# falcon-computing/bwa-flow

Measured on AMD Instinct MI355X. Metric: million reads/sec (2×150 bp PE) end-to-end align; SW-extend GCUPS at 1/2/4/8 MI355X, higher is better.
Workload: dtype int32

## Files before the change

bwa-flow_amd/csrc/capi.hip:

```cpp
#include <hip/hip_runtime.h>
#include <string.h>

#include <algorithm>
#include <chrono>
#include <cstdio>
#include <mutex>
#include <new>
#include <string>
#include <thread>
#include <vector>

#include "batch_host.h"
#include "ctx.h"
#include "engine.h"
#include "regpost.h"

using namespace bwagpu;

namespace {


__global__ void side_probe_spin(uint64_t ticks) {
  const uint64_t t0 = __builtin_amdgcn_s_memrealtime();
  while (__builtin_amdgcn_s_memrealtime() - t0 < ticks) __builtin_amdgcn_s_sleep(8);
// ... 118 lines not shown
  std::string why;
  if (!make_opt(opt, &ctx->opt, &why)) {
    delete ctx;
    return BWAGPU_E_INVAL;
  }
  ctx->device = device;
  ctx->opt_b = opt->b;
  ctx->ext_form = set_ext_form(-1);
  ctx->ext_short = ext_short_default();
  ctx->ext_short_fill = ext_short_fill_default();
  ctx->light_pack = light_pack_default();
  ctx->ungapped = ungapped_default();
  ctx->ungapped_right = ungapped_right_default();
  ctx->emu_finish = emu_finish_default();
  ctx->fused_launches = fused_launches_default();
  *made = ctx;
  HIPC(hipSetDevice(device), "hipSetDevice");
  HIPC(hipMalloc(&ctx->d_ann_off, sizeof(int64_t) * bns->n_seqs), "hipMalloc(ann_offset)");
  HIPC(hipMalloc(&ctx->d_ann_len, sizeof(int32_t) * bns->n_seqs), "hipMalloc(ann_len)");
  HIPC(hipMemcpy(ctx->d_ann_off, bns->ann_offset, sizeof(int64_t) * bns->n_seqs, hipMemcpyHostToDevice),
       "upload ann_offset");
  HIPC(hipMemcpy(ctx->d_ann_len, bns->ann_len, sizeof(int32_t) * bns->n_seqs, hipMemcpyHostToDevice),
       "upload ann_len");
  for (auto& s : ctx->slot) {
    HIPC(hipEventCreate(&s.ev0), "hipEventCreate");
    HIPC(hipEventCreate(&s.ev1), "hipEventCreate");
    HIPC(hipEventCreate(&s.ev2), "hipEventCreate");
    HIPC(hipEventCreate(&s.ev3), "hipEventCreate");
  }
  ctx->ref.l_pac = bns->l_pac;
// ... 174 lines not shown
  }();
  a.emu_strict = emu_strict;
  a.light_pack = ctx->light_pack;
  a.emu_finish = ctx->emu_finish;
  a.out = d_out;
  a.out_n = d_n;
  a.stats = d_stats;
  SpecStreams ss;
  HIPC(choose_side(ctx, s, st, &ss), "side stream");
  a.lq_bound = lq_max;
  const int tb = tb_bytes_for(ctx->opt, std::max(lq_max, 1));
  ss.form = ctx->ext_form;
  ss.short_q = ctx->ext_short;
  ss.short_fill = ctx->ext_short_fill;
  ss.fused = ctx->fused_launches;
  ss.pool = ctx->prof_ev.empty() ? nullptr : ctx->prof_ev.data();
  ss.pool_n = (int)ctx->prof_ev.size();
  ss.pool_used = &ctx->prof_used;
  HIPC(launch_spec_clear(a, db.n_reads, db.n_seeds, st), "spec clear");
  HIPC(launch_spec_chain2aln(ctx->opt, ctx->ref, db, a, tb, lq_max, st, ss), "spec chain2aln launch");
  return BWAGPU_OK;
}

}

int bwagpu::enqueue_chain2aln(bwagpu_ctx_t* ctx, Slot& s, const DevBatch& db, int lq_max, bwagpu_alnreg_t* d_out,
                              int32_t* d_n, int64_t* d_stats, hipStream_t st) {
  if (!use_read_kernels()) return enqueue_spec(ctx, s, db, lq_max, d_out, d_n, d_stats, st);
  ChainWin* win = nullptr;
  bwagpu_seed_t* prog = nullptr;
// ... 534 lines not shown

int bwagpu_ctx_emu_finish(bwagpu_ctx_t* ctx, int on) {
  if (!ctx) return BWAGPU_E_INVAL;
  const int prev = ctx->emu_finish;
  if (on >= 0) ctx->emu_finish = on ? 1 : 0;
  return prev;
}

int bwagpu_ctx_fused_launches(bwagpu_ctx_t* ctx, int mask) {
  if (!ctx) return BWAGPU_E_INVAL;
  const int prev = ctx->fused_launches;
  if (mask >= 0) ctx->fused_launches = mask & 7;
  return prev;
}

int bwagpu_debug_spec_finish(bwagpu_ctx_t* ctx, void* stream, int64_t* out) {
  if (!ctx || !out) return BWAGPU_E_INVAL;
  int32_t c[SPC_WORDS];
  if (int rc = spec_ctr_words(ctx, stream, c)) return rc;
  out[0] = c[SPC_FIN_NAR];
  out[1] = c[SPC_FIN_WIDE];
  out[2] = c[SPC_LIST_N];
  out[3] = c[SPC_LIGHT_N];
  return BWAGPU_OK;
}

int bwagpu_ctx_row_bound(bwagpu_ctx_t* ctx, int on) {
  if (!ctx) return BWAGPU_E_INVAL;
  const int prev = ctx->opt.row_bound;
  if (on >= 0) ctx->opt.row_bound = on ? 1 : 0;
  return prev;
}

int bwagpu_debug_ext_kernel(bwagpu_ctx_t* ctx, int32_t lq_max) {
  if (!ctx || lq_max < 1 || lq_max > BWAGPU_MAX_READ_LEN) return BWAGPU_E_INVAL;
  return ext_kernel_for(ctx->opt, ctx->ext_form, tb_bytes_for(ctx->opt, lq_max));
}

// ... 54 lines not shown
```

bwa-flow_amd/csrc/ctx.h:

```cpp
#pragma once
#include <hip/hip_runtime.h>
#include <stdint.h>

#include <algorithm>
#include <atomic>
#include <chrono>
#include <mutex>
#include <string>
#include <type_traits>
#include <vector>

#include "bwagpu.h"
#include "chain.h"
#include "engine.h"
#include "rescue.h"
#include "seed.h"
#include "stage_host.h"
#include "task_host.h"

namespace bwagpu {

inline std::atomic<int64_t> g_live_bufs{0}, g_live_bytes{0};

template <bool kPinned>
// ... 100 lines not shown
  bwagpu::DevOpt opt{};
  bwagpu::DevRef ref{};
  bool own_pac = false;
  void* d_pac = nullptr;
  int64_t* d_ann_off = nullptr;
  int32_t* d_ann_len = nullptr;
  int watchdog_ms = 10000;
  int ext_form = 0;
  int ext_short = 0;
  int light_pack = 0;
  int ext_short_fill = 0;
  int ungapped = 1;
  int ungapped_right = 1;
  int emu_finish = 1;
  int fused_launches = 5;
  Slot slot[BWAGPU_NUM_SLOTS];
  hipStream_t dev_stream[BWAGPU_NUM_SLOTS] = {};
  Slot dev_scratch[BWAGPU_NUM_SLOTS];
  DevBuf ex_tasks, ex_list, ex_q, ex_t, ex_res, ex_stats;
  DevBuf a2_tasks, a2_q, a2_t, a2_out, a2_scratch, a2_lists, a2_counts, a2_boff;
  DevBuf r2_tasks, r2_q, r2_out, r2_cig, r2_md, r2_lists, r2_z, r2_stats;
  DevBuf r2d_keys, r2d_lists, r2d_tab, r2d_z, r2d_sums;
  HostBuf r2d_htab;
  hipEvent_t r2d_done = nullptr, r2d_ev[2] = {};
  bool r2d_pending = false, r2d_timing = false, r2d_timed = false;
  double r2d_wait_ms = 0, r2d_call_ms = 0;
  int32_t r2d_jobs = 0;
  static constexpr int kA2Streams = 4;
  hipStream_t a2_st[kA2Streams] = {};
  hipEvent_t a2_fork = nullptr, a2_join[kA2Streams] = {};
// ... 198 lines not shown
```

bwa-flow_amd/csrc/engine.h:

```cpp
#pragma once
#include <hip/hip_runtime.h>
#include <stdint.h>

#include "bwagpu.h"
#include "bwagpu_debug.h"
#include "pure.h"
#include "spec_plan.h"
#include "ungapped.h"

namespace bwagpu {

struct ReadDesc {
  int64_t qoff;
  int32_t rd;
  int32_t lq;
  int32_t c0;
  int32_t nch;
  int32_t s0;
  int32_t ns;
};

struct ChainWin {
  int64_t lo, hi;
};
// ... 163 lines not shown
  int ext_prefetch;
  bwagpu_alnreg_t* out;
  int32_t* out_n;
  int64_t* stats;
};
struct SpecStreams {
  hipStream_t side = nullptr;
  hipEvent_t fork = nullptr, join = nullptr;
  hipEvent_t* pool = nullptr;
  int pool_n = 0;
  int* pool_used = nullptr;
  int form = 0;
  int short_q = 0;
  int short_fill = 0;
  int fused = 0;
};
enum {
  kFuseSort = 1,
  kFuseSettle = 2,
  kFuseHeavy = 4,
};
int fused_launches_default();
int ungapped_default();
int ungapped_right_default();
int emu_finish_default();
int set_ext_form(int form);
int ext_short_default();
int ext_short_fill_default();
int light_pack_default();
int ext_kernel_for(const DevOpt& o, int form, int tb_bytes);
hipError_t launch_spec_clear(const SpecArgs& a, int n_reads, int n_seeds, hipStream_t st);
hipError_t launch_spec_chain2aln(const DevOpt& o, const DevRef& ref, const DevBatch& b, const SpecArgs& a,
                                 int tb_bytes, int lq_max, hipStream_t st, const SpecStreams& ss);
size_t spec_select_lds(int tb_bytes);
int spec_redo_cap(int tb_bytes);

struct StreamTask {
// ... 27 lines not shown
```

bwa-flow_amd/csrc/spec.hip:

```cpp
#include "spec_dev.h"

namespace bwagpu {

__device__ uint32_t* g_trace = nullptr;
hipError_t set_trace_spec(void* p) { return hipMemcpyToSymbol(HIP_SYMBOL(g_trace), &p, sizeof(p)); }


__global__ void __launch_bounds__(256) spec_chain_kernel(DevOpt o, DevRef ref, DevBatch b, SpecArgs a) {
  sel_prio();
  const int c = blockIdx.x * blockDim.x + threadIdx.x;
  bool task = false, longc = false;
  int bin = 0, s0 = 0;
  if (c < b.n_chains) {
    const int rd = a.chain_read[c];
    s0 = b.chain_seed_off[c];
    const int ns = b.chain_seed_off[c + 1] - s0;
    const int lq = (int)(b.seq_off[rd + 1] - b.seq_off[rd]);
    if (ns <= 0) {
      a.win[c] = ChainWin{0, 0};
    } else {
      int64_t wlo = ref.l_pac << 1, whi = 0;
      longc = ns > kOrderLane;
      if (!longc) {
        uint64_t key[kOrderLane];
#pragma unroll
        for (int t = 0; t < kOrderLane; ++t) {
          key[t] = ~0ull;
          if (t < ns) {
            const bwagpu_seed_t v = b.seeds[s0 + t];
// ... 21 lines not shown
      } else {
        if (!longc) a.win[c] = ChainWin{wlo, whi};
        task = lq <= a.lq_bound;
        bin = spec_bin(lq);
      }
    }
  }
#pragma unroll
  for (int k = 0; k < kSpecBins; ++k) {
    const int p = wave_append(&a.ctr[SPC_CNT + k], task && bin == k);
    if (p >= 0) a.tasks[(size_t)k * b.n_chains + p] = make_int2(s0, c);
  }
  const int p = wave_append(&a.ctr[SPC_LONG_N], longc);
  if (p >= 0) a.longc[p] = c;
}

__global__ void __launch_bounds__(256) spec_reads_kernel(DevBatch b, SpecArgs a) {
  sel_prio();
  const int rd = blockIdx.x * blockDim.x + threadIdx.x;
  bool heavy = false;
  int ns = 0;
  if (rd < b.n_reads) {
    const int lq = (int)(b.seq_off[rd + 1] - b.seq_off[rd]);
    if (lq > a.lq_bound) atomicOr((unsigned long long*)&a.stats[ST_ERR], (unsigned long long)ERR_LEN);
    ReadDesc d;
    d.qoff = b.seq_off[rd];
    d.rd = rd;
    d.lq = lq;
    d.c0 = b.read_chain_off[rd];
    d.nch = b.read_chain_off[rd + 1] - d.c0;
    d.s0 = b.chain_seed_off[d.c0];
    d.ns = b.chain_seed_off[d.c0 + d.nch] - d.s0;
    a.rdesc[rd] = d;
    for (int c = d.c0; c < d.c0 + d.nch; ++c) a.chain_read[c] = rd;
    heavy = d.ns > kSelLight || d.nch > kSelLight;
    ns = d.ns;
  }
  const int p = wave_append(&a.ctr[SPC_HEAVY_N], heavy);
  if (p >= 0) {
    a.heavy[p] = rd;
    const long long words = 2 * tri_off(ns);
    int woff = -1, col = 0;
    if (ns <= kSelMatMaxSeeds) {
      const long long o = (long long)atomicAdd(reinterpret_cast<unsigned long long*>(&a.ctr[SPC_MATW64]),
                                               (unsigned long long)words);
      if (o + words <= a.mat_words) {
        woff = (int)o;
        col = atomicAdd(&a.ctr[SPC_HCOLS], ns);
        for (int i = 0; i < ns; ++i) a.colent[col + i] = p;
      }
    }
    a.hinfo[p] = make_int4(rd, woff, col, ns);
  }
}

constexpr int kOrderBlocks = 1024;
constexpr int kOrderLds = 4096;
__device__ __forceinline__ uint64_t order_key(const bwagpu_seed_t* sd, int i) {
  return (uint64_t)(uint32_t)sd[i].score << 32 | (uint32_t)i;
}
__global__ void __launch_bounds__(256) spec_order_kernel(DevOpt o, DevRef ref, DevBatch b, SpecArgs a) {
  sel_prio();
  __shared__ uint64_t keys[kOrderLds];
  __shared__ int64_t wred[2][4];
  const int tid = (int)threadIdx.x;
  const int n_long = __hip_atomic_load(&a.ctr[SPC_LONG_N], __ATOMIC_RELAXED, __HIP_MEMORY_SCOPE_AGENT);
  for (int gi = (int)blockIdx.x; gi < n_long; gi += (int)gridDim.x) {
// ... 2006 lines not shown
}
int emu_finish_default() {
  static const int on = [] {
    const char* e = getenv("BWAGPU_EMU_FINISH");
    return !(e && e[0] == '0');
  }();
  return on;
}
int fused_launches_default() {
  static const int m = [] {
    const char* e = getenv("BWAGPU_FUSED_LAUNCHES");
    return (e && e[0] ? atoi(e) : 5) & 7;
  }();
  return m;
}
int ext_short_fill_default() {
  static const int f = [] {
    const char* e = getenv("BWAGPU_EXT_SHORT_FILL");
    return std::min(std::max(e && e[0] ? atoi(e) : BWAGPU_EXT_SHORT_FILL_DEFAULT, 0), 100000);
  }();
  return f;
}


static void launch_sort(const ExtBin& k, const ExtRound& r, int bin0, int nbins, int short_q, int short_fill) {
  if (k.phased) launch_side_sort(r, bin0, nbins, short_q, short_fill);
  else launch_task_sort(r, bin0, nbins);
}
static void launch_ext_bin(const ExtBin& k, const ExtRound& r, int list, const ExtPlan& p, int short_fill) {
  if (k.family == SIDE4) launch_side_bin(k, r, list, p, short_fill);
// ... 15 lines not shown
  const bool prof = ss.pool && *ss.pool_used + 2 <= ss.pool_n;
  if (prof) (void)hipEventRecord(ss.pool[*ss.pool_used], st);
  launch_ext_bin(plan.bin[0], r, l + 0, plan, ss.short_fill);
  if (prof) {
    (void)hipEventRecord(ss.pool[*ss.pool_used + 1], st);
    *ss.pool_used += 2;
  }
  if (!bin1) return;
  launch_ext_bin(plan.bin[1], r, l + 1, plan, ss.short_fill);
  if (bin2) launch_task_long(r, l + 2);
}

hipError_t launch_spec_chain2aln(const DevOpt& o, const DevRef& ref, const DevBatch& b, const SpecArgs& a,
                                 int tb_bytes, int lq_max, hipStream_t st, const SpecStreams& ss) {
  if (b.n_reads == 0) return hipSuccess;
  hipLaunchKernelGGL(spec_reads_kernel, dim3((b.n_reads + 255) / 256), dim3(256), 0, st, b, a);
  if (b.n_chains) {
    hipLaunchKernelGGL(spec_chain_kernel, dim3((b.n_chains + 255) / 256), dim3(256), 0, st, o, ref, b, a);
    hipLaunchKernelGGL(spec_order_kernel, dim3(kOrderBlocks), dim3(256), 0, st, o, ref, b, a);
  }
  if (b.n_chains) {
    launch_ext_round(o, ref, b, a, 0, tb_bytes, lq_max, st, ss);
    launch_select<SEL_EMULATE>(o, ref, b, a, tb_bytes, st, ss);
    launch_ext_round(o, ref, b, a, 1, tb_bytes, lq_max, st, ss);
  }
  SpecArgs af = a;
  if (!b.n_chains) af.emu_finish = 0;
  launch_select<SEL_FINAL>(o, ref, b, af, tb_bytes, st, ss);
  if (b.n_chains && lq_max > kSpecBinLen[0] && !a.emu_strict) launch_ext_round(o, ref, b, a, 2, tb_bytes, lq_max, st, ss);
  if (b.n_chains) launch_select<SEL_REDO>(o, ref, b, a, tb_bytes, st, ss);
  return hipGetLastError();
}

__global__ void __launch_bounds__(256) spec_clear_kernel(SpecArgs a, int nr, int ns) {
  const int t0 = (int)(blockIdx.x * 256 + threadIdx.x), nt = (int)(gridDim.x * 256);
// ... 32 lines not shown
```

bwa-flow_amd/csrc/spec_side.hip:

```cpp
#include "side_sort.h"
#include "spec_dev.h"

namespace bwagpu {


struct UngSide {
  const uint8_t* rd;
  int64_t x0;
  int p0, d, qlen, lq;
};
__device__ __forceinline__ UngSeg ung_pass(const UngSide& s, const DevRef& ref, int base, const int8_t* mat,
                                           const int8_t* mat8, int max_mat) {
  const int last = min(base + 15, s.qlen - 1), cnt = last - base + 1;
  const int64_t two1 = (ref.l_pac << 1) - 1, pac_bytes = (ref.l_pac >> 2) + 1;
  const int64_t xa = s.x0 + (int64_t)s.d * base, xb = s.x0 + (int64_t)s.d * last;
  const bool rev = xa >= ref.l_pac;
  const int64_t fa = rev ? two1 - xa : xa, fb = rev ? two1 - xb : xb;
  UngSeg g;
  if (s.lq >= 16 && pac_bytes >= 8 && (xb >= ref.l_pac) == rev) {
    const int qa = s.p0 + s.d * base;
    const int ws = min(max(min(qa, qa + 15 * s.d), 0), s.lq - 16);
    const int64_t b0 = min(min(fa, fb) >> 2, pac_bytes - 8);
    uint64_t q[2], tw;
    __builtin_memcpy(q, s.rd + ws, 16);
// ... 380 lines not shown
    }
    __syncthreads();
#pragma unroll
    for (int m = 0; m < kPer; ++m) {
      if (kl[m] >= 0) foL[cnt[0][kl[m]] + rl[m]] = ft[m];
      if (kr[m] >= 0) foR[cnt[1][kr[m]] + rr[m]] = ft[m];
    }
    __syncthreads();
    for (int k = threadIdx.x; k < 2 * 256; k += 256) cnt[k >> 8][k & 255] = 0;
    __syncthreads();
  }
  if (threadIdx.x < 2 && ung[threadIdx.x])
    atomicAdd(&a.ctr[(threadIdx.x ? SPC_UNG_Q : SPC_UNG_N) + round], ung[threadIdx.x]);
}

__global__ void __launch_bounds__(256) spec_settle_right_kernel(DevOpt o, DevBatch b, SpecArgs a, int round, int bin0) {
  sel_prio();
  __shared__ int tot[2];
  __shared__ unsigned long long cel;
  if (threadIdx.x < 2) tot[threadIdx.x] = 0;
  if (threadIdx.x == 0) cel = 0;
  __syncthreads();
  const int list = round * kSpecBins + bin0 + (int)blockIdx.y;
  const int n = __hip_atomic_load(&a.ctr[SPC_CNT + list], __ATOMIC_RELAXED, __HIP_MEMORY_SCOPE_AGENT);
  const size_t off = spec_list_off(list, b.n_chains, b.n_seeds);
  int sides = 0, bases = 0;
  unsigned long long cells = 0;
  for (int i = (int)(blockIdx.x * 256 + threadIdx.x); i < n; i += (int)gridDim.x * 256) {
    const UngTask t = a.ungt[off + i];
    const int qb = (int)(t.qls & 1023u), ln = (int)((t.qls >> 10) & 1023u), lq = (int)(t.qls >> 20);
    if (!side_lists(a, off + i, qb, lq - qb - ln).late) continue;
    SeedExt e = a.ext[t.pos];
    settle_right(o, e, t.rbeg, qb, ln, lq, a.ung[off + i].side[1].s);
    e.w = max(e.w, o.w);
    e.calls += 2;
    a.ext[t.pos] = e;
    ++sides;
    bases += lq - qb - ln;
    cells += (unsigned long long)e.cells;
  }
  if (sides) {
    atomicAdd(&tot[0], sides);
    atomicAdd(&tot[1], bases);
    atomicAdd(&cel, cells);
  }
  __syncthreads();
  if (threadIdx.x < 2 && tot[threadIdx.x])
    atomicAdd(&a.ctr[(threadIdx.x ? SPC_UNGR_Q : SPC_UNGR_N) + round], tot[threadIdx.x]);
  if (threadIdx.x == 0 && cel) atomicAdd(reinterpret_cast<unsigned long long*>(a.ctr + SPC_SPEC64), cel);
}

struct SideTask {
  int64_t rbeg, qoff, rb;
  int32_t pos, dlo, dhi, qbeg, len, lq;
  int32_t tt, score, h0, truesc, qb, aw0, cells, rows, calls, pad_;
};
static_assert(sizeof(SideTask) <= 96, "SideTask layout");
typedef __attribute__((address_space(3))) SideTask LdsS;
#define SIDE_FIELDS(X) X(rbeg) X(qoff) X(rb) X(pos) X(dlo) X(dhi) X(qbeg) X(len) X(lq) X(tt) X(score) X(h0) \
  X(truesc) X(qb) X(aw0) X(cells) X(rows) X(calls)
__device__ __forceinline__ void spark(LdsS* p, const SideTask& t) {
#define X(f) p->f = t.f;
  SIDE_FIELDS(X)
#undef X
// ... 253 lines not shown
    if (hb) {
      SideTask t = sload(sb);
      if (side_advance<G, RIGHT>(t, o, a, xb, tlb, spec_cells)) hb = false;
      else spark(sb, t);
    }
#ifdef BWAGPU_OCC_DIAG
    tw[3] += __builtin_amdgcn_s_memtime() - c3;
#endif
  }
  return started;
}

template <int G, int PMAX, bool K8, bool RIGHT>
__global__ void __launch_bounds__(kBlock) spec_side4_kernel(DevOpt o, DevRef ref, DevBatch b, SpecArgs a, int list,
                                                            int tb_bytes, int wave_lds, int short_q, int tb_short,
                                                            int short_fill) {
  extern __shared__ __attribute__((aligned(16))) uint8_t lds[];
  uint8_t* const wlds = lds + (size_t)(threadIdx.x >> 6) * (size_t)wave_lds;
  const int n = uni(__hip_atomic_load(&a.ctr[(RIGHT ? SPC_RCNT : SPC_LCNT) + list], __ATOMIC_RELAXED,
                                      __HIP_MEMORY_SCOPE_AGENT));
  const FatTask* fl = (RIGHT ? a.ftaskR : a.ftask) + spec_list_off(list, b.n_chains, b.n_seeds);
  constexpr bool kShort = G == 16 && K8;
  int n_long = n;
  if constexpr (kShort) {
    if (short_q > 0) {
      n_long = min(n, uni(__hip_atomic_load(&a.ctr[(RIGHT ? SPC_RLONG : SPC_LLONG) + list], __ATOMIC_RELAXED,
                                            __HIP_MEMORY_SCOPE_AGENT)));
      const long long slots = (long long)gridDim.x * (kBlock / 64) * (128 / kShortG);
      if ((long long)(n - n_long) * 100 < slots * short_fill) n_long = n;
    }
  }
// ... 19 lines not shown
#endif
      if ((threadIdx.x & (kShortG - 1)) == 0 && ns) {
        atomicAdd(&a.ctr[SPC_SHORT_N], ns);
        atomicAdd(reinterpret_cast<unsigned long long*>(a.ctr + SPC_SPEC64), (unsigned long long)cells_s);
      }
    }
  }
#ifdef BWAGPU_OCC_DIAG
  if ((threadIdx.x & 63) == 0) {
    for (int k = 0; k < 8; ++k) atomicAdd(reinterpret_cast<unsigned long long*>(a.ctr + 32) + k, occ[k]);
    for (int k = 0; k < 4; ++k) atomicAdd(reinterpret_cast<unsigned long long*>(a.ctr + 48) + k, tw[k]);
  }
#endif
  if ((threadIdx.x & (G - 1)) == 0 && spec_cells)
    atomicAdd(reinterpret_cast<unsigned long long*>(a.ctr + SPC_SPEC64), (unsigned long long)spec_cells);
}


void launch_side_sort(const ExtRound& r, int bin0, int nbins, int short_q, int short_fill) {
  const int fuse = (r.ss.fused & kFuseSort) ? 1 : 0;
  if (r.a.ung)
    hipLaunchKernelGGL(spec_ungapped_kernel, dim3(512, nbins), dim3(256), 0, r.st, r.o, r.ref, r.b, r.a, r.round, bin0,
                       short_fill == 0 ? short_q : 0, fuse);
  if (!(fuse && r.a.ung)) hipLaunchKernelGGL(spec_sort2_count, dim3(256, nbins), dim3(256), 0, r.st, r.b, r.a, r.round, bin0);
  if (!fuse)
    hipLaunchKernelGGL(spec_sort2_scan, dim3(2 * nbins), dim3(256), 0, r.st, r.a, r.round, bin0, nbins, short_q);
  hipLaunchKernelGGL(spec_sort2_scatter, dim3(256, nbins), dim3(256), 0, r.st, r.o, r.b, r.a, r.round, bin0, short_q,
                     fuse);
}

template <int G, int PMAX, bool K8>
static void launch_side_pair(const ExtRound& r, int list, const ExtPlan& p, int short_fill) {
  const size_t lds = (size_t)(kBlock / 64) * p.wave_lds;
  const int nb = resident_blocks(spec_side4_kernel<G, PMAX, K8, false>, lds);
  const int gr = r.round == 2 ? std::min(nb, 64) : std::min(nb, ext2_grid(1 << 30, true));
  if (!(G == 16 && K8)) short_fill = 0;
  hipLaunchKernelGGL((spec_side4_kernel<G, PMAX, K8, false>), dim3(gr), dim3(kBlock), lds, r.st, r.o, r.ref, r.b, r.a,
                     list, r.tb_bytes, (int)p.wave_lds, p.short_q, p.tb_short, short_fill);
  const bool beside = r.a.ungt && r.ss.side && (r.ss.fused & kFuseSettle);
  if (beside) {
    (void)hipEventRecord(r.ss.fork, r.st);
    (void)hipStreamWaitEvent(r.ss.side, r.ss.fork, 0);
    hipLaunchKernelGGL(spec_settle_right_kernel, dim3(256, 1), dim3(256), 0, r.ss.side, r.o, r.b, r.a, r.round,
                       list % kSpecBins);
    (void)hipEventRecord(r.ss.join, r.ss.side);
  } else if (r.a.ungt) {
    hipLaunchKernelGGL(spec_settle_right_kernel, dim3(256, 1), dim3(256), 0, r.st, r.o, r.b, r.a, r.round,
                       list % kSpecBins);
  }
  hipLaunchKernelGGL((spec_side4_kernel<G, PMAX, K8, true>), dim3(gr), dim3(kBlock), lds, r.st, r.o, r.ref, r.b, r.a,
                     list, r.tb_bytes, (int)p.wave_lds, p.short_q, p.tb_short, short_fill);
  if (beside) (void)hipStreamWaitEvent(r.st, r.ss.join, 0);
}

void launch_side_bin(const ExtBin& k, const ExtRound& r, int list, const ExtPlan& p, int short_fill) {
  switch (ext_key(k.family, k.G, k.PMAX, k.K8)) {
    case ext_key(SIDE4, 16, 10, true): return launch_side_pair<16, 10, true>(r, list, p, short_fill);
    case ext_key(SIDE4, 32, 5, true): return launch_side_pair<32, 5, true>(r, list, p, short_fill);
    case ext_key(SIDE4, 32, 8, false): return launch_side_pair<32, 8, false>(r, list, p, short_fill);
    default: abort();
  }
}

}
```

bwa-flow_amd/python/bwagpu/abi.py:

```python
from __future__ import annotations

import ctypes as C
import os

import numpy as np

HERE = os.path.dirname(os.path.abspath(__file__))
PKG_ROOT = os.path.normpath(os.path.join(HERE, "..", ".."))
REPO_ROOT = os.path.normpath(os.path.join(PKG_ROOT, ".."))
LIB_DIR = os.path.join(PKG_ROOT, "lib")

ABI_VERSION = 1
OK, E_INVAL, E_NOMEM, E_DEVICE, E_HANG, E_RESULTS, E_UNSUPPORTED, E_NODEVICE = range(8)
ERR_NAMES = {
    OK: "OK", E_INVAL: "E_INVAL", E_NOMEM: "E_NOMEM", E_DEVICE: "E_DEVICE", E_HANG: "E_HANG",
    E_RESULTS: "E_RESULTS", E_UNSUPPORTED: "E_UNSUPPORTED", E_NODEVICE: "E_NODEVICE",
}
MAX_READ_LEN = 1023
NUM_SLOTS = 4

SEED_DTYPE = np.dtype([("rbeg", "<i8"), ("qbeg", "<i4"), ("len", "<i4"), ("score", "<i4"),
                       ("pad", "<i4")])
ALNREG_DTYPE = np.dtype([
    ("rb", "<i8"), ("re", "<i8"), ("qb", "<i4"), ("qe", "<i4"), ("rid", "<i4"), ("score", "<i4"),
# ... 178 lines not shown
    "bwagpu_set_device_read_len": (C.c_int, [_VP, C.c_int32]),
    "bwagpu_debug_ext_form": (C.c_int, [C.c_int]),
    "bwagpu_ctx_ext_form": (C.c_int, [_VP, C.c_int]),
    "bwagpu_ctx_ext_short": (C.c_int, [_VP, C.c_int]),
    "bwagpu_ctx_ext_short_fill": (C.c_int, [_VP, C.c_int]),
    "bwagpu_ctx_light_pack": (C.c_int, [_VP, C.c_int]),
    "bwagpu_debug_spec_short": (C.c_int, [_VP, _VP, _VP]),
    "bwagpu_ctx_row_bound": (C.c_int, [_VP, C.c_int]),
    "bwagpu_ctx_ungapped": (C.c_int, [_VP, C.c_int]),
    "bwagpu_debug_spec_ungapped": (C.c_int, [_VP, _VP, _VP]),
    "bwagpu_ctx_ungapped_right": (C.c_int, [_VP, C.c_int]),
    "bwagpu_debug_spec_ungapped_right": (C.c_int, [_VP, _VP, _VP]),
    "bwagpu_ctx_emu_finish": (C.c_int, [_VP, C.c_int]),
    "bwagpu_debug_spec_finish": (C.c_int, [_VP, _VP, _VP]),
    "bwagpu_ctx_fused_launches": (C.c_int, [_VP, C.c_int]),
    "bwagpu_debug_ext_kernel": (C.c_int, [_VP, C.c_int32]),
    "bwagpu_streams_concurrent": (C.c_int, [_VP, _VP]),
    "bwagpu_bwt_sa": (C.c_int, [_VP, C.c_int64, _VP, _VP]),
    "bwagpu_sw_stream": (C.c_int, [_VP, _VP, C.c_int64, _VP, C.c_int32, C.POINTER(C.c_int32)]),
    "bwagpu_collect_intv": (C.c_int, [_VP, C.POINTER(SeedOpt), C.c_int32, _VP, _VP, C.c_int32, _VP, C.c_int64,
                                       _VP]),
    "bwagpu_set_alt": (C.c_int, [_VP, _VP]),
    "bwagpu_seqs2chains": (C.c_int, [_VP, C.POINTER(SeedOpt), C.POINTER(ChainOpt), C.c_int32, _VP, _VP, C.c_int32,
                                      C.POINTER(ChainsC)]),
    "bwagpu_seqs2regions": (C.c_int, [_VP, C.POINTER(SeedOpt), C.POINTER(ChainOpt), C.c_int32, _VP, _VP, _VP,
                                       C.POINTER(_VP), C.POINTER(C.c_int64)]),
    "bwagpu_regs_post": (C.c_int, [_VP, C.POINTER(PostOpt), C.c_int32, C.c_int64, C.c_int32, _VP, _VP, _VP, _VP,
                                    _VP]),
    "bwagpu_regs_post_device": (C.c_int, [_VP, C.POINTER(PostOpt), C.c_int32, C.c_int64, C.POINTER(BatchC), _VP,
                                           _VP, _VP, _VP]),
# ... 24 lines not shown

def load() -> C.CDLL:
    global _lib
    if _lib is not None:
        return _lib
    p = lib_path()
    if os.environ.get("BWAGPU_NO_TORCH") != "1":
        try:
            import torch
        except Exception:
            pass
    if not os.path.exists(p):
        raise RuntimeError(f"bwagpu: HIP engine library missing at {p}; run __graft_entry__.build()")
    lib = C.CDLL(p)
    for name, (res, args) in PROTOS.items():
        if (name.startswith("bwagpu_debug_") or name in ("bwagpu_ctx_light_pack", "bwagpu_ctx_ungapped", "bwagpu_ctx_ungapped_right", "bwagpu_ctx_emu_finish", "bwagpu_ctx_fused_launches")) and not hasattr(lib, name):
            continue
        fn = getattr(lib, name)
        fn.restype = res
        fn.argtypes = args
    if lib.bwagpu_abi_version() != ABI_VERSION:
        raise RuntimeError("bwagpu: ABI version mismatch")
    _lib = lib
    return lib


def opt_from_dict(d: dict) -> Opt:
    o = Opt()
    for k in ("a", "b", "o_del", "e_del", "o_ins", "e_ins", "pen_clip5", "pen_clip3", "w", "zdrop"):
        setattr(o, k, int(d[k]))
    mat = d.get("mat")
# ... 19 lines not shown
```

bwa-flow_amd/python/bwagpu/engine.py:

```python
from __future__ import annotations

import ctypes as C
from dataclasses import dataclass

import numpy as np

from . import abi


class BwaGpuError(RuntimeError):
    def __init__(self, code: int, msg: str):
        super().__init__(f"{abi.ERR_NAMES.get(code, code)}: {msg}")
        self.code = code


def _ptr(a: np.ndarray | None):
    return None if a is None or a.size == 0 else a.ctypes.data_as(C.c_void_p)


@dataclass
class Batch:
    seq_off: np.ndarray
    seq: np.ndarray
    read_chain_off: np.ndarray
# ... 292 lines not shown
    def ungapped(self, on: int = -1) -> int:
        return self.lib.bwagpu_ctx_ungapped(self.ctx, int(on))

    def ungapped_right(self, on: int = -1) -> int:
        return self.lib.bwagpu_ctx_ungapped_right(self.ctx, int(on))

    def ungapped_right_counters(self, stream=None):
        out = np.zeros(6, np.int64)
        self._check(self.lib.bwagpu_debug_spec_ungapped_right(self.ctx, C.c_void_p(stream), _ptr(out)),
                    "debug_spec_ungapped_right")
        return out.reshape(3, 2)

    def fused_launches(self, mask: int = -1) -> int:
        return self.lib.bwagpu_ctx_fused_launches(self.ctx, int(mask))

    def emu_finish(self, on: int = -1) -> int:
        return self.lib.bwagpu_ctx_emu_finish(self.ctx, int(on))

    def row_bound(self, on: int = -1) -> int:
        return self.lib.bwagpu_ctx_row_bound(self.ctx, int(on))

    def set_device_read_len(self, max_len: int):
        self._check(self.lib.bwagpu_set_device_read_len(self.ctx, int(max_len)), "set_device_read_len")

    def sup_shift(self, shift: int):
        self._check(self.lib.bwagpu_debug_sup_shift(self.ctx, shift), "sup_shift")

    def seed_budget(self, budget: int):
        self._check(self.lib.bwagpu_debug_seed_budget(self.ctx, budget), "seed_budget")

# ... 233 lines not shown
```

include/bwagpu.h:

```cpp
#ifndef BWAGPU_H
#define BWAGPU_H

#include <stddef.h>
#include <stdint.h>

#ifdef __cplusplus
extern "C" {
#endif

#define BWAGPU_ABI_VERSION 1

enum {
  BWAGPU_OK = 0,
  BWAGPU_E_INVAL = 1,
  BWAGPU_E_NOMEM = 2,
  BWAGPU_E_DEVICE = 3,
  BWAGPU_E_HANG = 4,
  BWAGPU_E_RESULTS = 5,
  BWAGPU_E_UNSUPPORTED = 6,
  BWAGPU_E_NODEVICE = 7
};

#define BWAGPU_MAX_READ_LEN 1023
#define BWAGPU_NUM_SLOTS 4
// ... 168 lines not shown
int bwagpu_chain2aln_submit(bwagpu_ctx_t *ctx, int slot, const bwagpu_batch_t *batch);
int bwagpu_chain2aln_wait(bwagpu_ctx_t *ctx, int slot, bwagpu_alnreg_t *out_regs, int32_t *out_n);
int bwagpu_chain2aln(bwagpu_ctx_t *ctx, const bwagpu_batch_t *batch, bwagpu_alnreg_t *out_regs,
                     int32_t *out_n);

int bwagpu_chain2aln_stage(bwagpu_ctx_t *ctx, int slot, int32_t n_reads, int32_t n_chains, int32_t n_seeds,
                           int64_t seq_bytes, bwagpu_batch_t *view);
int bwagpu_chain2aln_results(bwagpu_ctx_t *ctx, int slot, const bwagpu_alnreg_t **regs, const int32_t **n);
int bwagpu_chain2aln_results_dense(bwagpu_ctx_t *ctx, int slot, const bwagpu_alnreg_t **regs, const int32_t **n,
                                   const int32_t **off);
int bwagpu_chain2aln_device(bwagpu_ctx_t *ctx, const bwagpu_batch_t *dev_batch,
                            bwagpu_alnreg_t *dev_out, int32_t *dev_n, int64_t *dev_stats,
                            void *stream);
int bwagpu_set_device_read_len(bwagpu_ctx_t *ctx, int32_t max_len);
int bwagpu_ctx_fused_launches(bwagpu_ctx_t *ctx, int mask);

int bwagpu_extend_batch(bwagpu_ctx_t *ctx, int32_t n_tasks, const bwagpu_ext_task_t *tasks,
                        const uint8_t *qpool, int64_t qpool_len, const uint8_t *tpool,
                        int64_t tpool_len, bwagpu_ext_result_t *results);

int bwagpu_align2_batch(bwagpu_ctx_t *ctx, int32_t n_tasks, const bwagpu_align2_task_t *tasks,
                        const uint8_t *qpool, int64_t qpool_len, const uint8_t *tpool, int64_t tpool_len,
                        bwagpu_kswr_t *results);
int bwagpu_align2_device(bwagpu_ctx_t *ctx, int32_t n_tasks, const bwagpu_align2_task_t *dev_tasks,
                         const uint8_t *dev_qpool, const uint8_t *dev_tpool, bwagpu_kswr_t *dev_results,
                         void *dev_scratch, void *stream);

int bwagpu_reg2aln_batch(bwagpu_ctx_t *ctx, int32_t n_tasks, const bwagpu_reg2aln_task_t *tasks,
                         const uint8_t *qpool, int64_t qpool_len, int32_t max_ops, int32_t max_md,
                         bwagpu_aln_t *out, uint32_t *cigar, char *md);
// ... 174 lines not shown
```

include/bwagpu_debug.h:

```cpp
#ifndef BWAGPU_DEBUG_H
#define BWAGPU_DEBUG_H
#include "bwagpu.h"

#ifdef __cplusplus
extern "C" {
#endif

int bwagpu_debug_seed_budget(bwagpu_ctx_t *ctx, int32_t budget);

int bwagpu_debug_sup_shift(bwagpu_ctx_t *ctx, int32_t shift);

int bwagpu_debug_set_trace(bwagpu_ctx_t *ctx, void *dev_ptr);
int bwagpu_debug_fail_wait(bwagpu_ctx_t *ctx, int after_n_waits, int code);
int bwagpu_debug_live_buffers(int64_t *n, int64_t *bytes);

int bwagpu_prof_start(bwagpu_ctx_t *ctx, int max_launches);
int bwagpu_debug_spec_counters(bwagpu_ctx_t *ctx, void *stream, int64_t *out);
int bwagpu_debug_occupancy(bwagpu_ctx_t *ctx, void *stream, int64_t *out);
int bwagpu_debug_spec_ext(bwagpu_ctx_t *ctx, void *stream, void *host_out, int32_t n);
int bwagpu_prof_read(bwagpu_ctx_t *ctx, double *total_ms, int32_t *launches);
int bwagpu_debug_ext_form(int form);
int bwagpu_ctx_ext_form(bwagpu_ctx_t *ctx, int form);
int bwagpu_ctx_ext_short(bwagpu_ctx_t *ctx, int q);
int bwagpu_ctx_ext_short_fill(bwagpu_ctx_t *ctx, int percent);
int bwagpu_ctx_light_pack(bwagpu_ctx_t *ctx, int on);
int bwagpu_debug_spec_short(bwagpu_ctx_t *ctx, void *stream, int64_t *out);
int bwagpu_ctx_ungapped(bwagpu_ctx_t *ctx, int on);
int bwagpu_debug_spec_ungapped(bwagpu_ctx_t *ctx, void *stream, int64_t *out);
int bwagpu_ctx_ungapped_right(bwagpu_ctx_t *ctx, int on);
int bwagpu_debug_spec_ungapped_right(bwagpu_ctx_t *ctx, void *stream, int64_t *out);
int bwagpu_ctx_emu_finish(bwagpu_ctx_t *ctx, int on);
int bwagpu_debug_spec_finish(bwagpu_ctx_t *ctx, void *stream, int64_t *out);
int bwagpu_ctx_row_bound(bwagpu_ctx_t *ctx, int on);
int bwagpu_debug_ext_kernel(bwagpu_ctx_t *ctx, int32_t lq_max);
int bwagpu_streams_concurrent(void *a, void *b);
int bwagpu_debug_rescue_drop(bwagpu_ctx_t *ctx, int32_t k);
int bwagpu_debug_rescue_times(bwagpu_ctx_t *ctx, double *out);
int bwagpu_debug_reg2aln_times(bwagpu_ctx_t *ctx, double *out);
int bwagpu_prof_intervals(bwagpu_ctx_t *ctx, double *start_ms, double *end_ms, int32_t max, int32_t *n);

#ifdef __cplusplus
}
#endif
#endif
```

tools_dev/trace_busy.py:

```python
import csv
import json
import sys
from collections import defaultdict


def union(iv):
    tot, cur_s, cur_e = 0, None, None
    for s, e in sorted(iv):
        if cur_e is None or s > cur_e:
            if cur_e is not None:
                tot += cur_e - cur_s
            cur_s, cur_e = s, e
        else:
            cur_e = max(cur_e, e)
    if cur_e is not None:
        tot += cur_e - cur_s
    return tot


def short(name):
    n = name.split("(")[0].replace("void ", "").replace("bwagpu::", "").replace("(anonymous namespace)::", "")
    return n


def load(path):
    rows = []
    for r in csv.DictReader(open(path)):
        rows.append(dict(name=short(r["Kernel_Name"]), q=int(r["Queue_Id"]), cid=int(r["Correlation_Id"]),
                         s=int(r["Start_Timestamp"]), e=int(r["End_Timestamp"])))
    rows.sort(key=lambda r: r["cid"])
    return rows


def sequences(rows):
    seqs, cur = [], None
    for r in rows:
        if r["name"] == "spec_reads_kernel":
            cur = []
            seqs.append(cur)
        if cur is not None and not r["name"].startswith("__amd"):
            cur.append(r)
    return seqs


def analyse(path, warmup=3, steps=20, kernel="spec_ext2_kernel<5>"):
    rows = load(path)
    seqs = sequences(rows)
    timed = [r for q in seqs[warmup:warmup + steps] for r in q]
    t0 = min(r["s"] for r in timed)
    t1 = max(r["e"] for r in timed)
    wall = (t1 - t0) / 1e6
    pre = kernel[:-1] + ", "
    k = [(r["s"], r["e"]) for r in timed if r["name"] == kernel or r["name"].startswith(pre)]
    per = 2 if any(r["name"].startswith(pre) for r in timed) else 1
    fam = defaultdict(list)
    for r in timed:
        fam[r["name"]].append((r["s"], r["e"]))
    out = {
        "trace": path, "sequences": len(seqs), "timed_steps": steps,
        "window_ms_per_step": round(wall / steps, 4),
        "gpu_busy_ms_per_step": round(union([(r["s"], r["e"]) for r in timed]) / 1e6 / steps, 4),
        "kernel": kernel, "launches": len(k),
        "kernel_sum_ms_per_step": round(sum(e - s for s, e in k) / 1e6 / steps, 4),
        "kernel_busy_ms_per_step": round(union(k) / 1e6 / steps, 4),
        "kernel_avg_launch_ms": round(sum(e - s for s, e in k) / 1e6 / max(len(k), 1), 4),
        "kernel_avg_pair_ms": round(per * sum(e - s for s, e in k) / 1e6 / max(len(k), 1), 4),
        "families_busy_ms_per_step": {n: round(union(v) / 1e6 / steps, 4)
                                      for n, v in sorted(fam.items(), key=lambda x: -union(x[1]))},
    }
    return out, seqs


def timeline(seqs, k):
    q = seqs[k]
# ... 20 lines not shown
```

Baseline: 75.93.

## Fold read and chain prep kernels into one launch and fold late settle into right-side kernel

Adds spec_prep_kernel, which does per-read descriptor setup and per-chain classification in a single launch. Each block stages read_chain_off in LDS, maps chains to reads by binary search and fills colent cooperatively, replacing the separate spec_reads_kernel and spec_chain_kernel launches. An optional kFoldLate mode runs the late right-settle pass as an epilogue of the right-side extension kernel instead of a separate or side-stream launch. Default mask 1 enables only the prep fold; it saves a launch and a global round trip for chain_read, at the cost of some load imbalance when a block's reads have many chains.

```diff
diff --git a/bwa-flow_amd/csrc/capi.hip b/bwa-flow_amd/csrc/capi.hip
--- a/bwa-flow_amd/csrc/capi.hip
+++ b/bwa-flow_amd/csrc/capi.hip
@@ -156,6 +156,7 @@
   ctx->ungapped_right = ungapped_right_default();
   ctx->emu_finish = emu_finish_default();
   ctx->fused_launches = fused_launches_default();
+  ctx->chain_folds = chain_folds_default();
   *made = ctx;
   HIPC(hipSetDevice(device), "hipSetDevice");
   HIPC(hipMalloc(&ctx->d_ann_off, sizeof(int64_t) * bns->n_seqs), "hipMalloc(ann_offset)");
@@ -360,6 +361,7 @@
   ss.short_q = ctx->ext_short;
   ss.short_fill = ctx->ext_short_fill;
   ss.fused = ctx->fused_launches;
+  ss.folds = ctx->chain_folds;
   ss.pool = ctx->prof_ev.empty() ? nullptr : ctx->prof_ev.data();
   ss.pool_n = (int)ctx->prof_ev.size();
   ss.pool_used = &ctx->prof_used;
@@ -924,6 +926,13 @@
   return prev;
 }
 
+int bwagpu_ctx_chain_folds(bwagpu_ctx_t* ctx, int mask) {
+  if (!ctx) return BWAGPU_E_INVAL;
+  const int prev = ctx->chain_folds;
+  if (mask >= 0) ctx->chain_folds = mask & 3;
+  return prev;
+}
+
 int bwagpu_debug_spec_finish(bwagpu_ctx_t* ctx, void* stream, int64_t* out) {
   if (!ctx || !out) return BWAGPU_E_INVAL;
   int32_t c[SPC_WORDS];
@@ -932,6 +941,17 @@
   out[1] = c[SPC_FIN_WIDE];
   out[2] = c[SPC_LIST_N];
   out[3] = c[SPC_LIGHT_N];
+  return BWAGPU_OK;
+}
+
+int bwagpu_debug_spec_prep(bwagpu_ctx_t* ctx, void* stream, int64_t* out) {
+  if (!ctx || !out) return BWAGPU_E_INVAL;
+  int32_t c[SPC_WORDS];
+  if (int rc = spec_ctr_words(ctx, stream, c)) return rc;
+  out[0] = c[SPC_HEAVY_N];
+  out[1] = c[SPC_HCOLS];
+  memcpy(&out[2], c + SPC_MATW64, 8);
+  out[3] = c[SPC_LONG_N];
   return BWAGPU_OK;
 }
 
diff --git a/bwa-flow_amd/csrc/ctx.h b/bwa-flow_amd/csrc/ctx.h
--- a/bwa-flow_amd/csrc/ctx.h
+++ b/bwa-flow_amd/csrc/ctx.h
@@ -138,6 +138,7 @@
   int ungapped_right = 1;
   int emu_finish = 1;
   int fused_launches = 5;
+  int chain_folds = 1;
   Slot slot[BWAGPU_NUM_SLOTS];
   hipStream_t dev_stream[BWAGPU_NUM_SLOTS] = {};
   Slot dev_scratch[BWAGPU_NUM_SLOTS];
diff --git a/bwa-flow_amd/csrc/engine.h b/bwa-flow_amd/csrc/engine.h
--- a/bwa-flow_amd/csrc/engine.h
+++ b/bwa-flow_amd/csrc/engine.h
@@ -201,6 +201,7 @@
   int short_q = 0;
   int short_fill = 0;
   int fused = 0;
+  int folds = 0;
 };
 enum {
   kFuseSort = 1,
@@ -208,6 +209,11 @@
   kFuseHeavy = 4,
 };
 int fused_launches_default();
+enum {
+  kFoldPrep = 1,
+  kFoldLate = 2,
+};
+int chain_folds_default();
 int ungapped_default();
 int ungapped_right_default();
 int emu_finish_default();
diff --git a/bwa-flow_amd/csrc/prep_map.h b/bwa-flow_amd/csrc/prep_map.h
--- /dev/null
+++ b/bwa-flow_amd/csrc/prep_map.h
@@ -0,0 +1,28 @@
+#pragma once
+#include <stdint.h>
+
+#ifdef __HIPCC__
+#define BWAGPU_PM_HD __host__ __device__
+#else
+#define BWAGPU_PM_HD
+#endif
+
+namespace bwagpu {
+
+constexpr int kPrepReads = 256;
+
+BWAGPU_PM_HD inline int prep_chain_read(const int32_t* off, int n, int32_t c) {
+  int lo = 0, hi = n;
+  while (hi - lo > 1) {
+    const int mid = (lo + hi) >> 1;
+    if (off[mid] <= c) lo = mid;
+    else hi = mid;
+  }
+  return lo;
+}
+
+BWAGPU_PM_HD inline int prep_passes(int32_t c0, int32_t c1, int width) {
+  return c1 > c0 ? (int)(((int64_t)c1 - c0 + width - 1) / width) : 0;
+}
+
+}
diff --git a/bwa-flow_amd/csrc/spec.hip b/bwa-flow_amd/csrc/spec.hip
--- a/bwa-flow_amd/csrc/spec.hip
+++ b/bwa-flow_amd/csrc/spec.hip
@@ -1,4 +1,5 @@
 #include "spec_dev.h"
+#include "prep_map.h"
 
 namespace bwagpu {
 
@@ -6,13 +7,11 @@
 hipError_t set_trace_spec(void* p) { return hipMemcpyToSymbol(HIP_SYMBOL(g_trace), &p, sizeof(p)); }
 
 
-__global__ void __launch_bounds__(256) spec_chain_kernel(DevOpt o, DevRef ref, DevBatch b, SpecArgs a) {
-  sel_prio();
-  const int c = blockIdx.x * blockDim.x + threadIdx.x;
+__device__ __forceinline__ void chain_lane(const DevOpt& o, const DevRef& ref, const DevBatch& b, const SpecArgs& a,
+                                           int c, int rd, bool in) {
   bool task = false, longc = false;
   int bin = 0, s0 = 0;
-  if (c < b.n_chains) {
-    const int rd = a.chain_read[c];
+  if (in) {
     s0 = b.chain_seed_off[c];
     const int ns = b.chain_seed_off[c + 1] - s0;
     const int lq = (int)(b.seq_off[rd + 1] - b.seq_off[rd]);
@@ -64,25 +63,29 @@
   const int p = wave_append(&a.ctr[SPC_LONG_N], longc);
   if (p >= 0) a.longc[p] = c;
 }
-
-__global__ void __launch_bounds__(256) spec_reads_kernel(DevBatch b, SpecArgs a) {
+__global__ void __launch_bounds__(256) spec_chain_kernel(DevOpt o, DevRef ref, DevBatch b, SpecArgs a) {
   sel_prio();
-  const int rd = blockIdx.x * blockDim.x + threadIdx.x;
+  const int c = blockIdx.x * blockDim.x + threadIdx.x;
+  const bool in = c < b.n_chains;
+  chain_lane(o, ref, b, a, c, in ? a.chain_read[c] : 0, in);
+}
+
+__device__ __forceinline__ int read_lane(const DevBatch& b, const SpecArgs& a, int rd, int c0, int c1, bool in,
+                                         int4& h) {
   bool heavy = false;
   int ns = 0;
-  if (rd < b.n_reads) {
+  if (in) {
     const int lq = (int)(b.seq_off[rd + 1] - b.seq_off[rd]);
     if (lq > a.lq_bound) atomicOr((unsigned long long*)&a.stats[ST_ERR], (unsigned long long)ERR_LEN);
     ReadDesc d;
     d.qoff = b.seq_off[rd];
     d.rd = rd;
     d.lq = lq;
-    d.c0 = b.read_chain_off[rd];
-    d.nch = b.read_chain_off[rd + 1] - d.c0;
-    d.s0 = b.chain_seed_off[d.c0];
-    d.ns = b.chain_seed_off[d.c0 + d.nch] - d.s0;
+    d.c0 = c0;
+    d.nch = c1 - c0;
+    d.s0 = b.chain_seed_off[c0];
+    d.ns = b.chain_seed_off[c1] - d.s0;
     a.rdesc[rd] = d;
-    for (int c = d.c0; c < d.c0 + d.nch; ++c) a.chain_read[c] = rd;
     heavy = d.ns > kSelLight || d.nch > kSelLight;
     ns = d.ns;
   }
@@ -97,10 +100,55 @@
       if (o + words <= a.mat_words) {
         woff = (int)o;
         col = atomicAdd(&a.ctr[SPC_HCOLS], ns);
-        for (int i = 0; i < ns; ++i) a.colent[col + i] = p;
-      }
-    }
-    a.hinfo[p] = make_int4(rd, woff, col, ns);
+      }
+    }
+    h = make_int4(rd, woff, col, ns);
+    a.hinfo[p] = h;
+  }
+  return p;
+}
+__global__ void __launch_bounds__(256) spec_reads_kernel(DevBatch b, SpecArgs a) {
+  sel_prio();
+  const int rd = blockIdx.x * blockDim.x + threadIdx.x;
+  const bool in = rd < b.n_reads;
+  const int c0 = in ? b.read_chain_off[rd] : 0, c1 = in ? b.read_chain_off[rd + 1] : 0;
+  int4 h = make_int4(0, -1, 0, 0);
+  const int p = read_lane(b, a, rd, c0, c1, in, h);
+  for (int c = c0; c < c1; ++c) a.chain_read[c] = rd;
+  if (p >= 0 && h.y >= 0)
+    for (int i = 0; i < h.w; ++i) a.colent[h.z + i] = p;
+}
+
+__global__ void __launch_bounds__(kPrepReads) spec_prep_kernel(DevOpt o, DevRef ref, DevBatch b, SpecArgs a) {
+  sel_prio();
+  __shared__ int32_t offs[kPrepReads + 1];
+  __shared__ int4 fill[kPrepReads];
+  __shared__ int n_fill;
+  const int tid = (int)threadIdx.x;
+  const int r0 = (int)blockIdx.x * kPrepReads;
+  offs[tid] = b.read_chain_off[min(r0 + tid, b.n_reads)];
+  if (tid == 0) {
+    offs[kPrepReads] = b.read_chain_off[min(r0 + kPrepReads, b.n_reads)];
+    n_fill = 0;
+  }
+  __syncthreads();
+  const int rd = r0 + tid;
+  int4 h = make_int4(0, -1, 0, 0);
+  const int p = read_lane(b, a, rd, offs[tid], offs[tid + 1], rd < b.n_reads, h);
+  if (p >= 0 && h.y >= 0 && h.w > 0) fill[atomicAdd(&n_fill, 1)] = make_int4(p, h.y, h.z, h.w);
+  __syncthreads();
+  for (int k = 0; k < n_fill; ++k) {
+    const int4 f = fill[k];
+    for (int i = tid; i < f.w; i += kPrepReads) a.colent[f.z + i] = f.x;
+  }
+  const int c0 = offs[0], c1 = offs[kPrepReads];
+  const int passes = prep_passes(c0, c1, kPrepReads);
+  for (int k = 0; k < passes; ++k) {
+    const int c = c0 + k * kPrepReads + tid;
+    const bool in = c < c1;
+    const int crd = in ? r0 + prep_chain_read(offs, kPrepReads, c) : 0;
+    if (in) a.chain_read[c] = crd;
+    chain_lane(o, ref, b, a, c, crd, in);
   }
 }
 
@@ -2137,6 +2185,13 @@
   }();
   return m;
 }
+int chain_folds_default() {
+  static const int m = [] {
+    const char* e = getenv("BWAGPU_CHAIN_FOLDS");
+    return (e && e[0] ? atoi(e) : 1) & 3;
+  }();
+  return m;
+}
 int ext_short_fill_default() {
   static const int f = [] {
     const char* e = getenv("BWAGPU_EXT_SHORT_FILL");
@@ -2182,11 +2237,15 @@
 hipError_t launch_spec_chain2aln(const DevOpt& o, const DevRef& ref, const DevBatch& b, const SpecArgs& a,
                                  int tb_bytes, int lq_max, hipStream_t st, const SpecStreams& ss) {
   if (b.n_reads == 0) return hipSuccess;
-  hipLaunchKernelGGL(spec_reads_kernel, dim3((b.n_reads + 255) / 256), dim3(256), 0, st, b, a);
-  if (b.n_chains) {
-    hipLaunchKernelGGL(spec_chain_kernel, dim3((b.n_chains + 255) / 256), dim3(256), 0, st, o, ref, b, a);
-    hipLaunchKernelGGL(spec_order_kernel, dim3(kOrderBlocks), dim3(256), 0, st, o, ref, b, a);
-  }
+  if (ss.folds & kFoldPrep) {
+    hipLaunchKernelGGL(spec_prep_kernel, dim3((b.n_reads + kPrepReads - 1) / kPrepReads), dim3(kPrepReads), 0, st, o,
+                       ref, b, a);
+  } else {
+    hipLaunchKernelGGL(spec_reads_kernel, dim3((b.n_reads + 255) / 256), dim3(256), 0, st, b, a);
+    if (b.n_chains)
+      hipLaunchKernelGGL(spec_chain_kernel, dim3((b.n_chains + 255) / 256), dim3(256), 0, st, o, ref, b, a);
+  }
+  if (b.n_chains) hipLaunchKernelGGL(spec_order_kernel, dim3(kOrderBlocks), dim3(256), 0, st, o, ref, b, a);
   if (b.n_chains) {
     launch_ext_round(o, ref, b, a, 0, tb_bytes, lq_max, st, ss);
     launch_select<SEL_EMULATE>(o, ref, b, a, tb_bytes, st, ss);
diff --git a/bwa-flow_amd/csrc/spec_side.hip b/bwa-flow_amd/csrc/spec_side.hip
--- a/bwa-flow_amd/csrc/spec_side.hip
+++ b/bwa-flow_amd/csrc/spec_side.hip
@@ -418,6 +418,28 @@
     atomicAdd(&a.ctr[(threadIdx.x ? SPC_UNG_Q : SPC_UNG_N) + round], ung[threadIdx.x]);
 }
 
+struct LateSums {
+  int sides, bases;
+  unsigned long long cells;
+};
+__device__ __forceinline__ LateSums settle_late_pass(const DevOpt& o, const SpecArgs& a, size_t off, int n, int i0,
+                                                     int stride) {
+  LateSums s{0, 0, 0};
+  for (int i = i0; i < n; i += stride) {
+    const UngTask t = a.ungt[off + i];
+    const int qb = (int)(t.qls & 1023u), ln = (int)((t.qls >> 10) & 1023u), lq = (int)(t.qls >> 20);
+    if (!side_lists(a, off + i, qb, lq - qb - ln).late) continue;
+    SeedExt e = a.ext[t.pos];
+    settle_right(o, e, t.rbeg, qb, ln, lq, a.ung[off + i].side[1].s);
+    e.w = max(e.w, o.w);
+    e.calls += 2;
+    a.ext[t.pos] = e;
+    ++s.sides;
+    s.bases += lq - qb - ln;
+    s.cells += (unsigned long long)e.cells;
+  }
+  return s;
+}
 __global__ void __launch_bounds__(256) spec_settle_right_kernel(DevOpt o, DevBatch b, SpecArgs a, int round, int bin0) {
   sel_prio();
   __shared__ int tot[2];
@@ -428,21 +450,9 @@
   const int list = round * kSpecBins + bin0 + (int)blockIdx.y;
   const int n = __hip_atomic_load(&a.ctr[SPC_CNT + list], __ATOMIC_RELAXED, __HIP_MEMORY_SCOPE_AGENT);
   const size_t off = spec_list_off(list, b.n_chains, b.n_seeds);
-  int sides = 0, bases = 0;
-  unsigned long long cells = 0;
-  for (int i = (int)(blockIdx.x * 256 + threadIdx.x); i < n; i += (int)gridDim.x * 256) {
-    const UngTask t = a.ungt[off + i];
-    const int qb = (int)(t.qls & 1023u), ln = (int)((t.qls >> 10) & 1023u), lq = (int)(t.qls >> 20);
-    if (!side_lists(a, off + i, qb, lq - qb - ln).late) continue;
-    SeedExt e = a.ext[t.pos];
-    settle_right(o, e, t.rbeg, qb, ln, lq, a.ung[off + i].side[1].s);
-    e.w = max(e.w, o.w);
-    e.calls += 2;
-    a.ext[t.pos] = e;
-    ++sides;
-    bases += lq - qb - ln;
-    cells += (unsigned long long)e.cells;
-  }
+  const LateSums ls = settle_late_pass(o, a, off, n, (int)(blockIdx.x * 256 + threadIdx.x), (int)gridDim.x * 256);
+  const int sides = ls.sides, bases = ls.bases;
+  const unsigned long long cells = ls.cells;
   if (sides) {
     atomicAdd(&tot[0], sides);
     atomicAdd(&tot[1], bases);
@@ -452,6 +462,24 @@
   if (threadIdx.x < 2 && tot[threadIdx.x])
     atomicAdd(&a.ctr[(threadIdx.x ? SPC_UNGR_Q : SPC_UNGR_N) + round], tot[threadIdx.x]);
   if (threadIdx.x == 0 && cel) atomicAdd(reinterpret_cast<unsigned long long*>(a.ctr + SPC_SPEC64), cel);
+}
+
+__device__ __forceinline__ void settle_late_epilogue(const DevOpt& o, const DevBatch& b, const SpecArgs& a, int list) {
+  const int n = __hip_atomic_load(&a.ctr[SPC_CNT + list], __ATOMIC_RELAXED, __HIP_MEMORY_SCOPE_AGENT);
+  const size_t off = spec_list_off(list, b.n_chains, b.n_seeds);
+  LateSums s = settle_late_pass(o, a, off, n, (int)(blockIdx.x * kBlock + threadIdx.x), (int)gridDim.x * kBlock);
+#pragma unroll
+  for (int m = 32; m >= 1; m >>= 1) {
+    s.sides += __shfl_xor(s.sides, m, 64);
+    s.bases += __shfl_xor(s.bases, m, 64);
+    s.cells += (unsigned long long)__shfl_xor((long long)s.cells, m, 64);
+  }
+  if ((threadIdx.x & 63) == 0 && s.sides) {
+    const int round = list / kSpecBins;
+    atomicAdd(&a.ctr[SPC_UNGR_N + round], s.sides);
+    atomicAdd(&a.ctr[SPC_UNGR_Q + round], s.bases);
+    if (s.cells) atomicAdd(reinterpret_cast<unsigned long long*>(a.ctr + SPC_SPEC64), s.cells);
+  }
 }
 
 struct SideTask {
@@ -735,7 +763,7 @@
 template <int G, int PMAX, bool K8, bool RIGHT>
 __global__ void __launch_bounds__(kBlock) spec_side4_kernel(DevOpt o, DevRef ref, DevBatch b, SpecArgs a, int list,
                                                             int tb_bytes, int wave_lds, int short_q, int tb_short,
-                                                            int short_fill) {
+                                                            int short_fill, int late) {
   extern __shared__ __attribute__((aligned(16))) uint8_t lds[];
   uint8_t* const wlds = lds + (size_t)(threadIdx.x >> 6) * (size_t)wave_lds;
   const int n = uni(__hip_atomic_load(&a.ctr[(RIGHT ? SPC_RCNT : SPC_LCNT) + list], __ATOMIC_RELAXED,
@@ -785,6 +813,9 @@
 #endif
   if ((threadIdx.x & (G - 1)) == 0 && spec_cells)
     atomicAdd(reinterpret_cast<unsigned long long*>(a.ctr + SPC_SPEC64), (unsigned long long)spec_cells);
+  if constexpr (RIGHT) {
+    if (late) settle_late_epilogue(o, b, a, list);
+  }
 }
 
 
@@ -807,9 +838,11 @@
   const int gr = r.round == 2 ? std::min(nb, 64) : std::min(nb, ext2_grid(1 << 30, true));
   if (!(G == 16 && K8)) short_fill = 0;
   hipLaunchKernelGGL((spec_side4_kernel<G, PMAX, K8, false>), dim3(gr), dim3(kBlock), lds, r.st, r.o, r.ref, r.b, r.a,
-                     list, r.tb_bytes, (int)p.wave_lds, p.short_q, p.tb_short, short_fill);
+                     list, r.tb_bytes, (int)p.wave_lds, p.short_q, p.tb_short, short_fill, 0);
   const bool beside = r.a.ungt && r.ss.side && (r.ss.fused & kFuseSettle);
-  if (beside) {
+  const bool fold = r.a.ungt && (r.ss.folds & kFoldLate) && !(r.ss.fused & kFuseSettle);
+  if (fold) {
+  } else if (beside) {
     (void)hipEventRecord(r.ss.fork, r.st);
     (void)hipStreamWaitEvent(r.ss.side, r.ss.fork, 0);
     hipLaunchKernelGGL(spec_settle_right_kernel, dim3(256, 1), dim3(256), 0, r.ss.side, r.o, r.b, r.a, r.round,
@@ -820,7 +853,7 @@
                        list % kSpecBins);
   }
   hipLaunchKernelGGL((spec_side4_kernel<G, PMAX, K8, true>), dim3(gr), dim3(kBlock), lds, r.st, r.o, r.ref, r.b, r.a,
-                     list, r.tb_bytes, (int)p.wave_lds, p.short_q, p.tb_short, short_fill);
+                     list, r.tb_bytes, (int)p.wave_lds, p.short_q, p.tb_short, short_fill, fold ? 1 : 0);
   if (beside) (void)hipStreamWaitEvent(r.st, r.ss.join, 0);
 }
 
diff --git a/bwa-flow_amd/python/bwagpu/abi.py b/bwa-flow_amd/python/bwagpu/abi.py
--- a/bwa-flow_amd/python/bwagpu/abi.py
+++ b/bwa-flow_amd/python/bwagpu/abi.py
@@ -216,6 +216,8 @@
     "bwagpu_ctx_emu_finish": (C.c_int, [_VP, C.c_int]),
     "bwagpu_debug_spec_finish": (C.c_int, [_VP, _VP, _VP]),
     "bwagpu_ctx_fused_launches": (C.c_int, [_VP, C.c_int]),
+    "bwagpu_ctx_chain_folds": (C.c_int, [_VP, C.c_int]),
+    "bwagpu_debug_spec_prep": (C.c_int, [_VP, _VP, _VP]),
     "bwagpu_debug_ext_kernel": (C.c_int, [_VP, C.c_int32]),
     "bwagpu_streams_concurrent": (C.c_int, [_VP, _VP]),
     "bwagpu_bwt_sa": (C.c_int, [_VP, C.c_int64, _VP, _VP]),
@@ -270,7 +272,7 @@
         raise RuntimeError(f"bwagpu: HIP engine library missing at {p}; run __graft_entry__.build()")
     lib = C.CDLL(p)
     for name, (res, args) in PROTOS.items():
-        if (name.startswith("bwagpu_debug_") or name in ("bwagpu_ctx_light_pack", "bwagpu_ctx_ungapped", "bwagpu_ctx_ungapped_right", "bwagpu_ctx_emu_finish", "bwagpu_ctx_fused_launches")) and not hasattr(lib, name):
+        if (name.startswith("bwagpu_debug_") or name in ("bwagpu_ctx_light_pack", "bwagpu_ctx_ungapped", "bwagpu_ctx_ungapped_right", "bwagpu_ctx_emu_finish", "bwagpu_ctx_fused_launches", "bwagpu_ctx_chain_folds")) and not hasattr(lib, name):
             continue
         fn = getattr(lib, name)
         fn.restype = res
diff --git a/bwa-flow_amd/python/bwagpu/engine.py b/bwa-flow_amd/python/bwagpu/engine.py
--- a/bwa-flow_amd/python/bwagpu/engine.py
+++ b/bwa-flow_amd/python/bwagpu/engine.py
@@ -330,6 +330,9 @@
     def fused_launches(self, mask: int = -1) -> int:
         return self.lib.bwagpu_ctx_fused_launches(self.ctx, int(mask))
 
+    def chain_folds(self, mask: int = -1) -> int:
+        return self.lib.bwagpu_ctx_chain_folds(self.ctx, int(mask))
+
     def emu_finish(self, on: int = -1) -> int:
         return self.lib.bwagpu_ctx_emu_finish(self.ctx, int(on))
 
diff --git a/include/bwagpu.h b/include/bwagpu.h
--- a/include/bwagpu.h
+++ b/include/bwagpu.h
@@ -206,6 +206,7 @@
                             void *stream);
 int bwagpu_set_device_read_len(bwagpu_ctx_t *ctx, int32_t max_len);
 int bwagpu_ctx_fused_launches(bwagpu_ctx_t *ctx, int mask);
+int bwagpu_ctx_chain_folds(bwagpu_ctx_t *ctx, int mask);
 
 int bwagpu_extend_batch(bwagpu_ctx_t *ctx, int32_t n_tasks, const bwagpu_ext_task_t *tasks,
                         const uint8_t *qpool, int64_t qpool_len, const uint8_t *tpool,
diff --git a/include/bwagpu_debug.h b/include/bwagpu_debug.h
--- a/include/bwagpu_debug.h
+++ b/include/bwagpu_debug.h
@@ -31,6 +31,7 @@
 int bwagpu_debug_spec_ungapped_right(bwagpu_ctx_t *ctx, void *stream, int64_t *out);
 int bwagpu_ctx_emu_finish(bwagpu_ctx_t *ctx, int on);
 int bwagpu_debug_spec_finish(bwagpu_ctx_t *ctx, void *stream, int64_t *out);
+int bwagpu_debug_spec_prep(bwagpu_ctx_t *ctx, void *stream, int64_t *out);
 int bwagpu_ctx_row_bound(bwagpu_ctx_t *ctx, int on);
 int bwagpu_debug_ext_kernel(bwagpu_ctx_t *ctx, int32_t lq_max);
 int bwagpu_streams_concurrent(void *a, void *b);
diff --git a/tools_dev/trace_busy.py b/tools_dev/trace_busy.py
--- a/tools_dev/trace_busy.py
+++ b/tools_dev/trace_busy.py
@@ -35,7 +35,7 @@
 def sequences(rows):
     seqs, cur = [], None
     for r in rows:
-        if r["name"] == "spec_reads_kernel":
+        if r["name"] in ("spec_reads_kernel", "spec_prep_kernel"):
             cur = []
             seqs.append(cur)
         if cur is not None and not r["name"].startswith("__amd"):
@@ -58,6 +58,7 @@
         fam[r["name"]].append((r["s"], r["e"]))
     out = {
         "trace": path, "sequences": len(seqs), "timed_steps": steps,
+        "launches_per_step": round(len(timed) / steps, 2),
         "window_ms_per_step": round(wall / steps, 4),
         "gpu_busy_ms_per_step": round(union([(r["s"], r["e"]) for r in timed]) / 1e6 / steps, 4),
         "kernel": kernel, "launches": len(k),
```

New measurement: 76.61 (median of 6 runs). About the same (+0.9%).
